# ska-sa/dc_sand

Hardware: AMD Instinct MI355X
Metric: Gcoeff/s (complex weights) 64ant x 1024beam x 32768chan per GPU (higher is better)
Workload: dtype f32

## Files before the change

### dc_sand_amd/csrc/bf_beamform_kernel.inc

```
template <int CH, bool WEIGHTED = false, class... Extra>
__global__ void __launch_bounds__(kBlock) bf_beamform_kernel(const bf_beamform_args a, const Extra... extra)
{
    static_assert(sizeof...(Extra) == (size_t)WEIGHTED && kernel_takes<bf_weights_args, Extra...> == WEIGHTED,
                  "the extra parameter is w, exactly where WEIGHTED is on");
    const bf_weights_args &w = kernel_extra<bf_weights_args>(extra...);
    extern __shared__ __attribute__((aligned(16))) float s_ant[];

    const uint32_t bid = blockIdx.x;
    const uint32_t bg = bid % a.n_bgroups;
    const uint32_t rest = bid / a.n_bgroups;
    const uint32_t cb = rest % a.n_cblocks;
    const uint32_t tex = rest / a.n_cblocks;

    const uint32_t b_local = threadIdx.x & 15u, t_in = threadIdx.x >> 4;
    const uint32_t b = bg * 16u + b_local;
    const uint32_t t = tex * 16u + t_in;
    const bool live = b < a.B;

    const uint32_t fw = a.flags[tex * 16u + (threadIdx.x & 15u)];
    const uint32_t fl = (fw >> 2) == a.epoch ? (fw & 3u) : DCS_CLASS_FAST_LOW;
    const int slow = __syncthreads_or((int)(fl == DCS_CLASS_SLOW));
    const int high = __syncthreads_or((int)(fl != DCS_CLASS_FAST_LOW));

    const float D = a.k.fDenominator, y = a.k.fRcpDenominator;
    const float *tp = a.terms + 2u * ((uint64_t)t * a.A * a.B + (live ? b : 0u));
    const float *gp = WEIGHTED ? w.gn + (live ? b : 0u) : nullptr;
    const uint32_t cbeg = cb * a.chan_per_block;
    const uint32_t cend = min(cbeg + a.chan_per_block, a.C);
    const uint32_t tex_g = a.tex0 + tex;
    const uint32_t words = a.A * 8u;
    const uint32_t sa = min(kAntChunk, a.A);

    for (uint32_t c = cbeg; c < cend; c += CH) {
        float fChan[CH], acc_re[CH], acc_im[CH];
#pragma unroll
        for (int h = 0; h < CH; h++) {
            fChan[h] = (float)(c + h);
            acc_re[h] = 0.0f;
            acc_im[h] = 0.0f;
        }
        for (uint32_t a0 = 0; a0 < a.A; a0 += kAntChunk) {
            const uint32_t na = min(kAntChunk, a.A - a0);
            const uint32_t cw = na * 8u;
            __syncthreads();
#pragma unroll
            for (int h = 0; h < CH; h++) {
                if (c + h < cend) {
                    const uint32_t *src = reinterpret_cast<const uint32_t *>(a.ant) +
                                          ((uint64_t)(c + h) * a.nt16_total + tex_g) * words + (uint64_t)a0 * 8u;
                    for (uint32_t i = threadIdx.x; i < cw; i += kBlock) {
                        const uint32_t w = src[i];
                        const floatx4 f = {(float)(int8_t)(w & 0xffu), (float)(int8_t)((w >> 8) & 0xffu),
                                           (float)(int8_t)((w >> 16) & 0xffu), (float)(int8_t)(w >> 24)};
                        *reinterpret_cast<floatx4 *>(&s_ant[((size_t)h * sa * 8u + i) * 4u]) = f;
                    }
                }
            }
            __syncthreads();

            auto sample = [&](int h, uint32_t al, float &sre, float &sim) {
                const floatx2 v = *reinterpret_cast<const floatx2 *>(&s_ant[(((size_t)h * sa + al) * 16u + t_in) * 2u]);
                sre = v.x;
                sim = v.y;
            };
            if (!slow) {
                dispatch_fast(a.k.uDiv3Exact != 0u, !high, [&](auto div3, auto lowdeg) {
                    auto terms_of = [&](uint32_t al) {
                        if constexpr (WEIGHTED) {
                            const uint64_t i = (uint64_t)(a0 + min(al, na - 1u)) * a.B;
                            const floatx2 k = *reinterpret_cast<const floatx2 *>(tp + 2u * i);
                            return floatx4{k.x, k.y, gp[i], 0.0f};
                        } else {
                            return *reinterpret_cast<const floatx2 *>(tp + 2u * (uint64_t)(a0 + min(al, na - 1u)) * a.B);
                        }
                    };
                    auto products = [&](uint32_t al, const auto kp) {
#pragma unroll
                        for (int h = 0; h < CH; h++) {
                            float re, im, sre, sim;
                            coeff_fast<decltype(div3)::value, decltype(lowdeg)::value>(kp.x, kp.y, fChan[h], D, y, re, im);
                            if constexpr (WEIGHTED) re = kp.z * re, im = kp.z * im;
                            sample(h, al, sre, sim);
                            const float pr = re * sre, pi = im * sim;
                            acc_re[h] = acc_re[h] + pr;
                            acc_im[h] = acc_im[h] + pi;
                        }
                    };
                    decltype(terms_of(0)) qa = terms_of(0), qb = terms_of(1), qc;
                    uint32_t al = 0;
                    for (; al + 2 < na; al += 3) {
                        qc = terms_of(al + 2);
                        products(al, qa);
                        qa = terms_of(al + 3);
                        products(al + 1, qb);
                        qb = terms_of(al + 4);
                        products(al + 2, qc);
                    }
                    if (al < na) products(al, qa);
                    if (al + 1 < na) products(al + 1, qb);
                });
            } else {
#pragma unroll
                for (int h = 0; h < CH; h++) {
                    float are = acc_re[h], aim = acc_im[h];
                    for (uint32_t al = 0; al < na; al++) {
                        const floatx2 kp = *reinterpret_cast<const floatx2 *>(tp + 2u * (uint64_t)(a0 + al) * a.B);
                        float re, im, sre, sim;
                        coeff_slow(kp.x, kp.y, fChan[h], D, re, im);
                        if constexpr (WEIGHTED) {
                            const float g = gp[(uint64_t)(a0 + al) * a.B];
                            re = g * re, im = g * im;
                        }
                        sample(h, al, sre, sim);
                        const float pr = re * sre, pi = im * sim;
                        are = are + pr;
                        aim = aim + pi;
                    }
                    acc_re[h] = are;
                    acc_im[h] = aim;
                }
            }
        }
        if (live) {
#pragma unroll
            for (int h = 0; h < CH; h++) {
                if (c + h < cend) {
                    floatx2 *dst = reinterpret_cast<floatx2 *>(a.beams) +
                                   (((uint64_t)(c + h) * a.nt16_total + tex_g) * a.B + b) * 16u + t_in;
                    if constexpr (WEIGHTED) {
                        const float sb = w.gs[b];
                        *dst = floatx2{sb * acc_re[h], sb * acc_im[h]};
                    } else {
                        *dst = floatx2{acc_re[h], acc_im[h]};
                    }
                }
            }
        }
    }
}
```

### dc_sand_amd/csrc/bf_capi.hip

```cpp

#include <cmath>
#include <cstdio>
#include <cstring>
#include <new>

#include "bf_host.h"

using namespace bf_host;

static_assert(sizeof(dcs_delay_vals) == 16, "delay_vals must be 4 x fp32 (BeamformerParameters.h:61-66)");

namespace {

bool params_ok(const dcs_bf_params *p)
{
    if (!p) return false;
    if (p->nr_channels < 1 || p->nr_channels > (1 << 24)) return false;
    if (p->nr_stations < 1 || p->nr_beams < 1) return false;
    if ((uint64_t)p->nr_stations * (uint64_t)p->nr_beams > 0x7fffffffull) return false;
    if (!(p->sampling_period > 0.0f) || !std::isfinite(p->sampling_period)) return false;
    if (p->fft_size < 1) return false;
    if (p->nr_samples_per_channel < 1 || p->accumulations_before_new_coeffs < 1) return false;
    if (!(p->adc_sample_rate > 0.0) || !std::isfinite(p->adc_sample_rate)) return false;
    const float D = p->sampling_period * (float)p->nr_channels;
// ... 271 lines not shown
        if ((st = (int)bf_warm_module_incoherent()) != 0) break;
        if ((st = (int)bf_warm_module_filterbank()) != 0) break;
        if ((st = (int)bf_warm_module_stokes()) != 0) break;
        if ((st = (int)bf_warm_module_dedisperse()) != 0) break;
        if ((st = (int)bf_warm_module_single_pulse()) != 0) break;
        if ((st = (int)bf_warm_module_correlator()) != 0) break;
        if ((st = (int)bf_warm_module_ddc()) != 0) break;
        const size_t tb = (size_t)c->n_pairs * sizeof(dcs_delay_vals);
        if ((st = (int)hipMalloc((void **)&c->d_table[0], tb)) != 0) break;
        if ((st = (int)hipMalloc((void **)&c->d_table[1], tb)) != 0) break;
        const size_t db = (size_t)kDtSlots * kDtSlotFloats * sizeof(float);
        if ((st = (int)hipMalloc((void **)&c->d_dt, db)) != 0) break;
        if ((st = (int)hipMalloc((void **)&c->d_tt_terms, (size_t)kTermsInline * c->pairs_pad * 8u)) != 0) break;
        if ((st = (int)hipMalloc((void **)&c->d_tt_flags, (size_t)kTermsInline * (c->pairs_pad / 64u) * 4u)) != 0) break;
        if ((st = (int)hipHostMalloc((void **)&c->h_dt, db, hipHostMallocDefault)) != 0) break;
        for (int i = 0; i < kDtSlots && st == 0; i++) st = (int)hipEventCreateWithFlags(&c->dt_ev[i], hipEventDisableTiming);
        if (st != 0) break;
        for (int i = 0; i < kSideStreams && st == 0; i++) {
            st = (int)hipStreamCreateWithFlags(&c->side[i], hipStreamNonBlocking);
            if (st == 0) st = (int)hipEventCreateWithFlags(&c->join_ev[i], hipEventDisableTiming);
        }
        if (st == 0) st = (int)hipEventCreateWithFlags(&c->fork_ev, hipEventDisableTiming);
        if (st != 0) break;
        c->h_dt[0] = 0.0f;
        if ((st = (int)hipMemcpy(c->d_dt, c->h_dt, sizeof(float), hipMemcpyHostToDevice)) != 0) break;
        if ((st = verify_div3(&c->k)) != 0) break;
        c->div3_verified = c->k.uDiv3Exact;
        for (int w = 0; w < 2; w++) {
            bf_kernel_launch l;
            const uint32_t nt_all = (uint32_t)(c->p.nr_samples_per_channel < (int)kDtInline ? c->p.nr_samples_per_channel : (int)kDtInline);
            float dts[kDtInline] = {0.0f};
            if (prepare_tiled(c, w == 1, nullptr, 0.0f, nt_all > 0 ? nt_all : 1u, 0, (uint32_t)c->p.nr_channels, nullptr, &l, dts, false) == DCS_OK && l.func) {
                hipFuncAttributes attr;
                (void)hipFuncGetAttributes(&attr, l.func);
            }
        }
    } while (0);
    if (st != 0) {
        dcs_bf_destroy(c);
        return st;
    }
    *out = c;
    return DCS_OK;
}

int dcs_bf_destroy(dcs_bf_context *c)
{
    if (!c) return DCS_OK;
    (void)hipFree(c->d_table[0]);
    (void)hipFree(c->d_table[1]);
    (void)hipFree(c->d_dt);
    (void)hipFree(c->d_terms);
    (void)hipFree(c->d_flags);
    (void)hipFree(c->d_wnorm);
    (void)hipFree(c->d_wscale);
    (void)hipFree(c->d_tt_terms);
    (void)hipFree(c->d_tt_flags);
    if (c->h_dt) (void)hipHostFree(c->h_dt);
    for (int i = 0; i < kDtSlots; i++)
        if (c->dt_ev[i]) (void)hipEventDestroy(c->dt_ev[i]);
    for (int i = 0; i < kSideStreams; i++) {
        if (c->join_ev[i]) (void)hipEventDestroy(c->join_ev[i]);
        if (c->side[i]) (void)hipStreamDestroy(c->side[i]);
    }
    if (c->fork_ev) (void)hipEventDestroy(c->fork_ev);
    delete c;
    return DCS_OK;
}

int dcs_bf_upload_delays(dcs_bf_context *c, const dcs_delay_vals *table, void *stream)
{
    if (!c || !table) return DCS_ERR_INVALID_ARGUMENT;
    DCS_CHECK_DEVICE(c);
    const int nxt = c->table_set ? (c->cur ^ 1) : c->cur;
    DCS_TRY(hipMemcpyAsync(c->d_table[nxt], table, (size_t)c->n_pairs * sizeof(dcs_delay_vals),
                           hipMemcpyHostToDevice, as_stream(stream)));
    c->cur = nxt;
    c->table_set = true;
    return DCS_OK;
}

int dcs_bf_set_delays_from_global(dcs_bf_context *c, const void *d_global, uint32_t nb_total,
                                  uint32_t beam_offset, void *stream)
{
    if (!c || !d_global) return DCS_ERR_INVALID_ARGUMENT;
    DCS_CHECK_DEVICE(c);
    if ((uint64_t)beam_offset + (uint64_t)c->p.nr_beams > nb_total) return DCS_ERR_OUT_OF_RANGE;
    if ((reinterpret_cast<uintptr_t>(d_global) & 15u) != 0) return DCS_ERR_INVALID_ARGUMENT;
    const int nxt = c->table_set ? (c->cur ^ 1) : c->cur;
    DCS_TRY(bf_launch_gather_beams(c->d_table[nxt], static_cast<const dcs_delay_vals *>(d_global),
                                   (uint32_t)c->p.nr_stations, (uint32_t)c->p.nr_beams, nb_total, beam_offset,
                                   as_stream(stream)));
    c->cur = nxt;
    c->table_set = true;
    return DCS_OK;
}

int dcs_bf_set_tuning(dcs_bf_context *c, const dcs_bf_tuning *t)
{
    if (!c) return DCS_ERR_INVALID_ARGUMENT;
    if (!t) {
        std::memset(&c->tune, 0, sizeof(c->tune));
        c->tune.nontemporal = -1;
        c->tune.xcd_remap = -1;
        c->tune.rows_same_tile = -1;
        c->k.uDiv3Exact = c->div3_verified;
        c->k.fLowDegLimit = 500.0f;
        c->k.uHalfMath = 0u;
        std::memset(c->tuned, 0, sizeof(c->tuned));
        return DCS_OK;
    }
    if (t->form < 0 || t->form > 3) return DCS_ERR_INVALID_ARGUMENT;
    if (t->nontemporal < -1 || t->nontemporal > 1) return DCS_ERR_INVALID_ARGUMENT;
    if (t->chan_per_block < 0 || t->chan_per_block > (1 << 24)) return DCS_ERR_INVALID_ARGUMENT;
    if (t->tiles_per_block != 0 && t->tiles_per_block != 1 && t->tiles_per_block != 2 && t->tiles_per_block != 4)
        return DCS_ERR_INVALID_ARGUMENT;
    if (t->waves_per_block != 0 && t->waves_per_block != 4 && t->waves_per_block != 8 && t->waves_per_block != 16)
        return DCS_ERR_INVALID_ARGUMENT;
    if (t->rows_per_wave < 0 || t->rows_per_wave > 4) return DCS_ERR_INVALID_ARGUMENT;
    if (t->rows_same_tile < -1 || t->rows_same_tile > 1) return DCS_ERR_INVALID_ARGUMENT;
    if (t->xcd_remap < -1 || t->xcd_remap > 1) return DCS_ERR_INVALID_ARGUMENT;
    if (t->math_mode < 0 || t->math_mode > 15) return DCS_ERR_INVALID_ARGUMENT;
    if ((t->math_mode & 4) && t->nontemporal == 0) return DCS_ERR_UNSUPPORTED;
    if (t->wg_per_cu < -1 || t->wg_per_cu == 1 || t->wg_per_cu > 7) return DCS_ERR_INVALID_ARGUMENT;
    c->tune = *t;
    c->k.uDiv3Exact = (t->math_mode & 1) ? 0u : c->div3_verified;
    c->k.fLowDegLimit = (t->math_mode & 2) ? 0.0f : 500.0f;
    c->k.uHalfMath = (t->math_mode & 4) ? 1u : 0u;
    return DCS_OK;
}

int dcs_bf_gpu_utilisation(const dcs_bf_params *p, float kernel_ms, float out[2])
{
    if (!params_ok(p) || !out) return DCS_ERR_INVALID_ARGUMENT;
    const float fRateOfFFTs_Hz = ((float)p->adc_sample_rate) / ((float)p->fft_size);
    const float fTransferTimePerPacket_s = 1 / fRateOfFFTs_Hz;
    float single = (kernel_ms / 1000.0) / (p->nr_samples_per_channel * fTransferTimePerPacket_s);
    float multiple = single / ((float)p->accumulations_before_new_coeffs);
    single *= 4;
    multiple *= 4;
    out[0] = single;
    out[1] = multiple;
    return DCS_OK;
}

#ifdef DCS_PROBES
int dcs_probe_set_knobs(dcs_bf_context *c, const dcs_probe_knobs *k)
{
    if (!c) return DCS_ERR_INVALID_ARGUMENT;
    if (!k) {
        std::memset(&c->probe, 0, sizeof(c->probe));
        return DCS_OK;
    }
    if (k->pace < 0 || k->pace > 4096 || k->fail_at_step < 0) return DCS_ERR_INVALID_ARGUMENT;
    c->probe = *k;
    return DCS_OK;
}
#endif

}
```

### dc_sand_amd/csrc/bf_capi_beamform.hip

```cpp

#include <cstdlib>
#include <cstring>

#include "bf_host.h"

using namespace bf_host;

namespace {

int next_flag_epoch(dcs_bf_context *c, hipStream_t s, uint32_t *epoch)
{
    if (c->flag_epoch >= (1u << 30) - 2u) {
        DCS_TRY(bf_launch_clear_words(c->d_flags, c->terms_steps * (c->pairs_pad / 64u), s));
        c->flag_epoch = 0;
    }
    *epoch = ++c->flag_epoch;
    return DCS_OK;
}

int clear_class_words(dcs_bf_context *c, uint32_t nt, hipStream_t s)
{
    if (!c->flags_cleared) {
        hipStreamCaptureStatus cs = hipStreamCaptureStatusNone;
        DCS_TRY(hipStreamIsCapturing(s, &cs));
        if (cs == hipStreamCaptureStatusNone) return DCS_OK;
        c->flags_cleared = true;
    }
    DCS_TRY(bf_launch_clear_words(c->d_flags, nt, s));
    return DCS_OK;
}

}

namespace bf_host {

int ensure_terms(dcs_bf_context *c, hipStream_t stream)
{
    if (c->d_terms && c->d_flags) return DCS_OK;
    {
        const int cap = refuse_if_capturing(stream);
        if (cap != DCS_OK) return cap;
    }
    if (!c->d_terms) DCS_TRY(hipMalloc((void **)&c->d_terms, (size_t)c->terms_steps * c->pairs_pad * 8u));
    if (!c->d_flags) {
        const size_t nb = (size_t)c->terms_steps * (c->pairs_pad / 64u) * 4u;
        DCS_TRY(hipMalloc((void **)&c->d_flags, nb));
        DCS_TRY(bf_launch_clear_words(c->d_flags, (uint32_t)(nb / 4u), stream));
        c->flag_epoch = 0;
    }
    return DCS_OK;
}

}

namespace {
int ensure_weights(dcs_bf_context *c, hipStream_t stream)
{
    if (c->d_wnorm && c->d_wscale) return DCS_OK;
    {
        const int cap = refuse_if_capturing(stream);
        if (cap != DCS_OK) return cap;
    }
    if (!c->d_wnorm) DCS_TRY(hipMalloc((void **)&c->d_wnorm, (size_t)c->n_pairs * sizeof(float)));
    if (!c->d_wscale) DCS_TRY(hipMalloc((void **)&c->d_wscale, (size_t)c->p.nr_beams * sizeof(float)));
    return DCS_OK;
}

int launch_bform_terms(dcs_bf_context *c, const float *d_weights, uint32_t nt, const float *dt_dev, float dt0, const float *dt_inline,
                       hipStream_t s, uint32_t *epoch)
{
    const int st_ep = next_flag_epoch(c, s, epoch);
    if (st_ep != DCS_OK) return st_ep;
    const int st_clr = clear_class_words(c, nt, s);
    if (st_clr != DCS_OK) return st_clr;
    bf_bform_terms_args ta;
    std::memset(&ta, 0, sizeof(ta));
    ta.delays = c->d_table[c->cur];
    ta.terms = c->d_terms;
    ta.flags = c->d_flags;
    ta.epoch = *epoch;
    ta.dt_dev = dt_dev;
    ta.dt0 = dt0;
    ta.n_pairs = c->n_pairs;
    ta.A = (uint32_t)c->p.nr_stations;
    ta.B = (uint32_t)c->p.nr_beams;
    ta.nt = nt;
    ta.k = c->k;
    const bf_weights_args wa = {d_weights, c->d_wnorm, c->d_wscale};
    return (int)(d_weights ? bf_launch_bform_terms_weighted(ta, wa, dt_inline, s) : bf_launch_bform_terms(ta, dt_inline, s));
}

int beamform_impl(dcs_bf_context *c, const dt_source &src, uint32_t nt, const int8_t *d_antenna,
                  size_t antenna_bytes, float *d_beams, size_t beams_bytes, void *stream, const float *d_weights = nullptr)
{
    if (!c || (nt && (!d_antenna || !d_beams))) return DCS_ERR_INVALID_ARGUMENT;
    DCS_CHECK_DEVICE(c);
    if (nt % 16u) return DCS_ERR_INVALID_ARGUMENT;
    if (!c->table_set) return DCS_ERR_NOT_READY;
    const uint32_t A = (uint32_t)c->p.nr_stations, B = (uint32_t)c->p.nr_beams, C = (uint32_t)c->p.nr_channels;
    if (antenna_bytes < (size_t)A * C * nt * 2u) return DCS_ERR_INVALID_ARGUMENT;
    if (beams_bytes < (size_t)B * C * nt * 2u * sizeof(float)) return DCS_ERR_INVALID_ARGUMENT;
    if ((reinterpret_cast<uintptr_t>(d_antenna) & 3u) || (reinterpret_cast<uintptr_t>(d_beams) & 7u))
        return DCS_ERR_INVALID_ARGUMENT;
    {
        const int st_range = check_dt_range(c, src, nt);
        if (st_range != DCS_OK) return st_range;
    }
    hipStream_t s = as_stream(stream);
    {
        int st_alloc = ensure_terms(c, s);
        if (st_alloc == DCS_OK && d_weights) st_alloc = ensure_weights(c, s);
        if (st_alloc != DCS_OK) return st_alloc;
    }
    const bf_weights_args wa = {d_weights, c->d_wnorm, c->d_wscale};
    uint32_t chunk = c->terms_steps & ~15u;
    if (chunk > kDtSlotFloats) chunk = kDtSlotFloats;
    if (chunk == 0) return DCS_ERR_UNSUPPORTED;
    if (nt > kDtInline) {
        const int cap = refuse_if_capturing(s);
        if (cap != DCS_OK) return cap;
    }
    for (uint32_t done = 0; done < nt;) {
        const uint32_t n = (nt - done) < chunk ? (nt - done) : chunk;
        const float *dt_dev = nullptr;
        float dt_val[kDtInline];
        const bool inl = n <= kDtInline;
        int st = inl ? fill_dt(c, src, done, n, dt_val) : stage_dt(c, src, done, n, s, &dt_dev);
        if (st != DCS_OK) return st;
        uint32_t epoch = 0;
        st = launch_bform_terms(c, d_weights, n, dt_dev, 0.0f, inl ? dt_val : nullptr, s, &epoch);
        if (st != DCS_OK) return st;
        bf_beamform_args a;
        std::memset(&a, 0, sizeof(a));
        a.terms = c->d_terms;
        a.flags = c->d_flags;
        a.epoch = epoch;
        a.ant = d_antenna;
        a.beams = d_beams;
        a.A = A;
        a.B = B;
        a.C = C;
        a.nt16 = n / 16u;
        a.tex0 = done / 16u;
        a.nt16_total = nt / 16u;
        uint32_t cpb = 4;
        while (cpb > 1 && (uint64_t)((B + 15u) / 16u) * ((C + cpb - 1) / cpb) * a.nt16 < 2048u) cpb >>= 1;
        a.chan_per_block = cpb;
        a.k = c->k;
        DCS_TRY(bf_launch_beamform(a, d_weights ? &wa : nullptr, s));
        done += n;
    }
    return DCS_OK;
}
}

namespace {
struct bacc_output {
    enum { kFloat, kInt8, kBlockPower } kind;
    const float *d_weights;
    bf_quant_args quant;
    const bf_complex_args *complex = nullptr;
    size_t block_bytes() const
    {
        return kind == kBlockPower ? sizeof(float) : 32u * (kind == kInt8 ? sizeof(int8_t) : sizeof(float));
    }
    uintptr_t align_mask() const { return kind == kBlockPower ? 3u : 7u; }
};

int beamform_acc_impl(dcs_bf_context *c, const dt_source &src, uint32_t nt, const int8_t *d_antenna, size_t antenna_bytes,
                      void *d_beams, size_t beams_bytes, void *stream, const bacc_output &out = {bacc_output::kFloat, nullptr, {}})
{
    if (!c || (nt && (!d_antenna || !d_beams))) return DCS_ERR_INVALID_ARGUMENT;
    DCS_CHECK_DEVICE(c);
    if (nt % 16u) return DCS_ERR_INVALID_ARGUMENT;
    if (!c->table_set) return DCS_ERR_NOT_READY;
    const uint32_t A = (uint32_t)c->p.nr_stations, B = (uint32_t)c->p.nr_beams, C = (uint32_t)c->p.nr_channels;
    if (A > 256u) return DCS_ERR_UNSUPPORTED;
    if (antenna_bytes < (size_t)A * C * nt * 2u) return DCS_ERR_INVALID_ARGUMENT;
    if (beams_bytes < (size_t)B * C * (nt / 16u) * out.block_bytes()) return DCS_ERR_INVALID_ARGUMENT;
    if ((reinterpret_cast<uintptr_t>(d_antenna) & 15u) || (reinterpret_cast<uintptr_t>(d_beams) & out.align_mask()))
        return DCS_ERR_INVALID_ARGUMENT;
    if ((out.d_weights || out.kind != bacc_output::kFloat || out.complex) && (c->tune.math_mode & 8)) return DCS_ERR_UNSUPPORTED;
    if (nt == 0) return DCS_OK;
    {
        const int st_range = check_dt_range(c, src, 1);
        if (st_range != DCS_OK) return st_range;
    }
    hipStream_t s = as_stream(stream);
    {
        int st_alloc = ensure_terms(c, s);
        if (st_alloc == DCS_OK && out.d_weights) st_alloc = ensure_weights(c, s);
        if (st_alloc != DCS_OK) return st_alloc;
    }
    float dt_coeff = 0.0f;
    int st = fill_dt(c, src, 0, 1, &dt_coeff);
    if (st != DCS_OK) return st;
    uint32_t epoch = 0;
    st = launch_bform_terms(c, out.d_weights, 1, nullptr, dt_coeff, nullptr, s, &epoch);
    if (st != DCS_OK) return st;
    bf_bacc_args a;
    std::memset(&a, 0, sizeof(a));
    a.terms = c->d_terms;
    a.flags = c->d_flags;
    a.epoch = epoch;
    a.ant = d_antenna;
    a.beams = static_cast<float *>(d_beams);
    a.A = A;
    a.B = B;
    a.C = C;
    a.nT16 = nt / 16u;
    a.k = c->k;
    a.fp32_chain = (c->tune.math_mode & 8) ? 1u : 0u;
#ifdef DCS_PROBES
    auto knob = [](int32_t v, const char *env) { const char *e = std::getenv(env); return (uint32_t)(v ? v : (e ? std::atoi(e) : 0)); };
    a.max_rounds = knob(c->probe.bacc_rounds, "DCS_BACC_ROUNDS");
    a.probe = knob(c->probe.bacc_probe, "DCS_BACC_PROBE");
    a.unstaged = knob(c->probe.bacc_unstaged, "DCS_BACC_UNSTAGED");
    a.plain_stores = knob(c->probe.bacc_plain, "DCS_BACC_PLAIN");
    a.no_share = knob(c->probe.bacc_no_share, "DCS_BACC_NOSHARE");
    a.wg_per_cu = knob(c->probe.bacc_wg_per_cu, "DCS_BACC_WPC");
    a.order = knob(c->probe.bacc_order, "DCS_BACC_ORDER");
    a.nbt_force = knob(c->probe.bacc_nbt, "DCS_BACC_NBT");
    a.nw_force = knob(c->probe.bacc_waves, "DCS_BACC_WAVES");
#endif
    const bf_weights_args wa = {out.d_weights, c->d_wnorm, c->d_wscale};
    return (int)bf_launch_beamform_acc(a, out.d_weights ? &wa : nullptr, out.kind == bacc_output::kInt8 ? &out.quant : nullptr,
                                       out.kind == bacc_output::kBlockPower, out.complex, s);
}

}

namespace bf_host {

int generate_and_beamform_weighted_impl(dcs_bf_context *c, const float *dt, uint64_t t0, uint32_t nt, const int8_t *d_antenna,
                                        size_t antenna_bytes, const float *d_weights, float *d_beams, size_t beams_bytes,
                                        void *stream)
{
    if (int e = generate_and_beamform_weighted_args(c, dt, t0, nt, d_weights)) return e;
    return beamform_impl(c, dt_or_index(dt, t0), nt, d_antenna, antenna_bytes, d_beams, beams_bytes, stream, d_weights);
}

int beamform_accumulated_weighted_impl(dcs_bf_context *c, const float *dt_coeff, uint64_t t_coeff, uint32_t nt,
                                       const int8_t *d_antenna, size_t antenna_bytes, const float *d_weights, float *d_beams,
                                       size_t beams_bytes, void *stream)
{
    if (int e = beamform_accumulated_weighted_args(c, nt, d_weights)) return e;
    return beamform_acc_impl(c, dt_or_index(dt_coeff, t_coeff), nt, d_antenna, antenna_bytes, d_beams, beams_bytes,
                             stream, {bacc_output::kFloat, d_weights, {}});
}

int beamform_accumulated_q8_impl(dcs_bf_context *c, const float *dt_coeff, uint64_t t_coeff, uint32_t nt, const int8_t *d_antenna,
                                 size_t antenna_bytes, const float *d_weights, const float *d_quant_gains, int8_t *d_beams_q8,
                                 size_t beams_bytes, unsigned long long *d_clip_count, void *stream)
{
    if (int e = beamform_accumulated_q8_args(c, nt, d_weights, d_quant_gains, d_clip_count)) return e;
    return beamform_acc_impl(c, dt_or_index(dt_coeff, t_coeff), nt, d_antenna, antenna_bytes, d_beams_q8, beams_bytes,
                             stream, {bacc_output::kInt8, d_weights, {d_quant_gains, d_clip_count}});
}

int beamform_accumulated_power_impl(dcs_bf_context *c, const float *dt_coeff, uint64_t t_coeff, uint32_t nt, const int8_t *d_antenna,
                                    size_t antenna_bytes, const float *d_weights, float *d_block_power, size_t power_bytes,
                                    void *stream)
{
    if (int e = beamform_accumulated_power_args(c, nt, d_weights, d_block_power)) return e;
    return beamform_acc_impl(c, dt_or_index(dt_coeff, t_coeff), nt, d_antenna, antenna_bytes, d_block_power, power_bytes,
                             stream, {bacc_output::kBlockPower, d_weights, {}});
}

int beamform_accumulated_complex_impl(dcs_bf_context *c, const float *dt_coeff, uint64_t t_coeff, uint32_t nt, const int8_t *d_antenna,
                                      size_t antenna_bytes, const float *d_weights, uint32_t flags, float *d_beams, size_t beams_bytes,
                                      void *stream)
{
    if (int e = beamform_accumulated_complex_args(c, nt, d_weights, flags, d_beams)) return e;
    const bf_complex_args cx = {flags & DCS_BF_COMPLEX_CONJ};
    return beamform_acc_impl(c, dt_or_index(dt_coeff, t_coeff), nt, d_antenna, antenna_bytes, d_beams, beams_bytes, stream,
                             {bacc_output::kFloat, d_weights, {}, &cx});
}

int beamform_accumulated_complex_power_impl(dcs_bf_context *c, const float *dt_coeff, uint64_t t_coeff, uint32_t nt,
                                            const int8_t *d_antenna, size_t antenna_bytes, const float *d_weights, uint32_t flags,
                                            float *d_block_power, size_t power_bytes, void *stream)
{
    if (int e = beamform_accumulated_complex_power_args(c, nt, d_weights, flags, d_block_power)) return e;
    const bf_complex_args cx = {flags & DCS_BF_COMPLEX_CONJ};
    return beamform_acc_impl(c, dt_or_index(dt_coeff, t_coeff), nt, d_antenna, antenna_bytes, d_block_power, power_bytes, stream,
                             {bacc_output::kBlockPower, d_weights, {}, &cx});
}

int beamform_accumulated_complex_q8_impl(dcs_bf_context *c, const float *dt_coeff, uint64_t t_coeff, uint32_t nt,
                                         const int8_t *d_antenna, size_t antenna_bytes, const float *d_weights, uint32_t flags,
                                         const float *d_quant_gains, int8_t *d_beams_q8, size_t beams_bytes,
                                         unsigned long long *d_clip_count, void *stream)
{
    if (int e = beamform_accumulated_complex_q8_args(c, nt, d_weights, flags, d_quant_gains, d_beams_q8, d_clip_count)) return e;
    const bf_complex_args cx = {flags & DCS_BF_COMPLEX_CONJ};
    return beamform_acc_impl(c, dt_or_index(dt_coeff, t_coeff), nt, d_antenna, antenna_bytes, d_beams_q8, beams_bytes, stream,
                             {bacc_output::kInt8, d_weights, {d_quant_gains, d_clip_count}, &cx});
}
// ... 33 lines not shown
```

### dc_sand_amd/csrc/bf_kernels.h

```cpp
#ifndef DCS_BF_KERNELS_H
#define DCS_BF_KERNELS_H

#include <hip/hip_runtime.h>
#include <stdint.h>

#include "bf_math.h"

struct bf_tiled_args {
    const dcs_delay_vals *delays;
    void *out;
    const float *dt_dev;
    float dt0;
    uint32_t n_pairs;
    uint32_t c0, nc;
    uint32_t nt;
    uint32_t chan_per_block;
    uint32_t n_tile_groups;
    uint32_t n_cblocks;
    uint32_t xcd_remap;
#ifdef DCS_PROBES
    uint32_t pace;
#endif
    dcs_bf_consts k;
    const float *terms;
    const uint32_t *flags;
    uint32_t pairs_pad;
};
constexpr uint32_t kDtInline = 256;
struct bf_tiled_args_inl {
    bf_tiled_args a;
    float dt_inline[kDtInline];
};

struct bf_kernel_launch {
    const void *func;
    dim3 grid, block;
    uint32_t shared;
    bf_tiled_args_inl args;
};
hipError_t bf_prepare_tiled(const bf_tiled_args &a, const float *dt_inline, bool out16, int tiles_per_block,
                            bool nontemporal, bf_kernel_launch *out);

struct bf_terms_args {
    const dcs_delay_vals *delays;
    float *terms;
    uint32_t *flags;
    const float *dt_dev;
    float dt0;
    uint32_t n_pairs, pairs_pad, nt;
    dcs_bf_consts k;
    float dt_inline[8];
    void *out;
    uint32_t c0, nc, out16;
};
constexpr uint32_t kTermsInline = 8;
hipError_t bf_launch_terms(const bf_terms_args &a, hipStream_t stream);
hipError_t bf_prepare_terms(const bf_terms_args &a, const void **func, dim3 *grid, dim3 *block);

struct bf_rows_args {
    const float *terms;
    const uint32_t *flags;
    void *out;
    uint32_t n_pairs, pairs_pad;
    uint32_t c0, nc, nt;
    uint32_t n_colgroups, n_rowgroups;
    uint32_t xcd_remap;
    uint32_t div3;
    uint32_t same_tile;
#ifdef DCS_PROBES
    uint32_t pace;
#endif
    uint32_t lds_pad;
    float D, y;
};
hipError_t bf_launch_rows(const bf_rows_args &a, bool out16, int waves_per_block, int rows_per_wave,
                          bool nontemporal, bool xcd_remap, bool nomath, hipStream_t stream);

struct bf_bform_terms_args {
    const dcs_delay_vals *delays;
    float *terms;
    uint32_t *flags;
    uint32_t epoch;
    const float *dt_dev;
    float dt0;
    uint32_t n_pairs, A, B, nt;
    dcs_bf_consts k;
};
struct bf_bform_terms_args_inl {
    bf_bform_terms_args a;
    float dt_inline[kDtInline];
};
hipError_t bf_launch_bform_terms(const bf_bform_terms_args &a, const float *dt_inline, hipStream_t stream);

struct bf_weights_args {
    const float *g;
    float *gn;
    float *gs;
};
hipError_t bf_launch_clear_words(uint32_t *words, uint32_t n, hipStream_t stream);
hipError_t bf_launch_bform_terms_weighted(const bf_bform_terms_args &a, const bf_weights_args &w, const float *dt_inline,
                                          hipStream_t stream);

struct bf_beamform_args {
    const float *terms;
    const uint32_t *flags;
    uint32_t epoch;
    const int8_t *ant;
    float *beams;
    uint32_t A, B, C;
    uint32_t nt16;
    uint32_t tex0;
    uint32_t nt16_total;
    uint32_t chan_per_block;
    uint32_t n_bgroups, n_cblocks;
    dcs_bf_consts k;
};
hipError_t bf_launch_beamform(const bf_beamform_args &a, const bf_weights_args *w, hipStream_t stream);

struct bf_bacc_args {
    const float *terms;
    const uint32_t *flags;
    uint32_t epoch;
    const int8_t *ant;
    float *beams;
    uint32_t A, B, C, nT16;
    uint32_t fp32_chain;
    uint32_t share_off;
#ifdef DCS_PROBES
    uint32_t max_rounds;
    uint32_t no_share;
    uint32_t plain_stores;
    uint32_t wg_per_cu;
    uint32_t unstaged;
    uint32_t order;
    uint32_t nbt_force;
    uint32_t nw_force;
    uint32_t probe;
#endif
    uint32_t tiles_per_wg, n_bgroups, n_tgroups, nbt_log2, xcd_group;
    dcs_bf_consts k;
};
__host__ __device__ inline uint32_t bf_xcd_grouped(uint32_t w, uint32_t total, uint32_t G)
{
    if (G <= 1u) return w;
    const uint32_t full = total - total % (8u * G);
    if (w >= full) return w;
    const uint32_t x = w & 7u, q = w >> 3;
    return ((q / G) * 8u + x) * G + q % G;
}

#ifdef DCS_PROBES
#define BACC_KNOB(a, f) ((a).f)
#else
#define BACC_KNOB(a, f) 0u
#endif
struct bf_quant_args {
    const float *gains;
    unsigned long long *clips;
};
struct bf_complex_args {
    uint32_t conj;
};
hipError_t bf_launch_beamform_acc(const bf_bacc_args &a, const bf_weights_args *w, const bf_quant_args *q, bool power,
                                  const bf_complex_args *cx, hipStream_t stream);
hipError_t bf_warm_module_mfma();

struct bf_incoh_args {
    const int8_t *ant;
    const float *weights;
    uint32_t *block_power;
    uint64_t rows;
    uint64_t n_groups;
    uint32_t A;
};
hipError_t bf_launch_incoherent_power(const bf_incoh_args &a, hipStream_t stream);
hipError_t bf_warm_module_incoherent();

struct bf_stokes_args {
    const int8_t *beams_x;
    const int8_t *beams_y;
    int32_t *block_stokes;
    uint64_t rows;
    uint64_t n_groups;
    uint32_t nr_stokes;
};
hipError_t bf_launch_stokes_block(const bf_stokes_args &a, hipStream_t stream);
hipError_t bf_warm_module_stokes();

enum bf_integrate_type { BF_INTEGRATE_F32, BF_INTEGRATE_U32 , BF_INTEGRATE_I32 };
struct bf_integrate_args {
    const void *blocks;
    float *out;
    uint64_t total;
    uint32_t bs;
    uint32_t C;
    uint32_t nr_blocks;
    uint32_t n;
    uint32_t accumulate;
};
hipError_t bf_launch_integrate(bf_integrate_type type, const bf_integrate_args &a, hipStream_t stream);
hipError_t bf_warm_module_integrate();

struct bf_dmdelay_args {
    const double *dms;
    int32_t *delays;
    uint64_t total;
    uint32_t C;
    double freq_first, freq_step, sample_time;
};
hipError_t bf_launch_dm_delays(const bf_dmdelay_args &a, hipStream_t stream);
struct bf_dedisp_args {
    const uint8_t *in;
    const int32_t *delays;
    const uint8_t *mask;
    uint32_t *out;
    uint64_t in_spectra, first, out_spectra, first_out;
    uint32_t C, B, T, nr_dm, max_delay;
    uint32_t t_tiles, dm_tiles;
};
hipError_t bf_launch_dedisperse(const bf_dedisp_args &a, hipStream_t stream);
hipError_t bf_warm_module_dedisperse();

struct bf_dtsums_args {
    const uint32_t *plane;
    uint64_t *sums;
    uint64_t plane_spectra, first;
    uint32_t T;
    uint32_t accumulate;
};
hipError_t bf_launch_dm_time_sums(const bf_dtsums_args &a, uint64_t series, hipStream_t stream);
struct bf_boxcar_args {
    const uint32_t *plane;
    const uint32_t *widths;
    uint32_t *peaks;
    uint64_t plane_spectra, first, peak_blocks, first_block;
    uint32_t T, nr_widths, max_width, block_len;
    uint32_t run;
    uint32_t segments;
};
hipError_t bf_launch_boxcar_peaks(const bf_boxcar_args &a, uint64_t series, hipStream_t stream);
struct bf_peaksnr_args {
    const uint32_t *peaks;
    const uint32_t *widths;
    const uint64_t *sums;
    float *snr;
    uint32_t *best;
    uint64_t peak_blocks, first_block, count;
    uint64_t total;
    uint32_t nr_blocks, nr_widths, max_width;
};
hipError_t bf_launch_peak_snr(const bf_peaksnr_args &a, hipStream_t stream);
hipError_t bf_warm_module_single_pulse();

struct bf_corr_args {
    const int8_t *ant;
    int32_t *vis;
    uint64_t NB;
    uint64_t items;
    uint32_t A;
    uint32_t C;
    uint32_t nT16;
    uint32_t n;
    uint32_t nr_vis;
    uint32_t tiles;
    uint32_t st;
    uint32_t units;
// ... 88 lines not shown
```

### dc_sand_amd/csrc/bf_kernels.hip

```cpp

#include "bf_kernels.h"

#include <hip/hip_runtime.h>

#include <cstring>
#include <type_traits>

#include "bf_device.h"

namespace {

template <bool OUT16, int TPB, bool NT, bool ALIGNED, bool NOMATH, int TAG = 0, bool INL = false, bool TERMS = false, bool HALF = false>
__global__ void __launch_bounds__(kBlock) bf_tiled_kernel(const std::conditional_t<INL, bf_tiled_args_inl, bf_tiled_args> args)
{
    const bf_tiled_args &a = [&]() -> const bf_tiled_args & {
        if constexpr (INL)
            return args.a;
        else
            return args;
    }();
    constexpr int PPL = OUT16 ? 4 : 2;
    constexpr int TILE = 64 * PPL;
    constexpr int ROWS = 4 / TPB;
    constexpr uint32_t EB = OUT16 ? 4u : 8u;
// ... 649 lines not shown
}

template <bool OUT16>
hipError_t launch_rows_o(const bf_rows_args &a, int nw, int rpw, bool nt, bool aligned, bool nomath, dim3 grid,
                         hipStream_t stream)
{
    switch (nw) {
    case 4: return launch_rows_w<OUT16, 4>(a, rpw, nt, aligned, nomath, grid, stream);
    case 8: return launch_rows_w<OUT16, 8>(a, rpw, nt, aligned, nomath, grid, stream);
    case 16: return launch_rows_w<OUT16, 16>(a, rpw, nt, aligned, nomath, grid, stream);
    default: return hipErrorInvalidValue;
    }
}

}

hipError_t bf_prepare_terms(const bf_terms_args &a, const void **func, dim3 *grid, dim3 *block)
{
    *func = nullptr;
    if (a.nt == 0 || a.pairs_pad == 0) return hipSuccess;
    if (a.pairs_pad % kBlock || a.nt > 65535u) return hipErrorInvalidValue;
    if (a.dt_dev == nullptr && a.nt > kTermsInline) return hipErrorInvalidValue;
    *func = reinterpret_cast<const void *>(&bf_terms_kernel);
    *grid = dim3(a.pairs_pad / kBlock, a.nt);
    *block = dim3(kBlock);
    return hipSuccess;
}

hipError_t bf_launch_terms(const bf_terms_args &a, hipStream_t stream)
{
    const void *func;
    dim3 grid, block;
    const hipError_t e = bf_prepare_terms(a, &func, &grid, &block);
    if (e != hipSuccess || func == nullptr) return e;
    void *params[] = {const_cast<bf_terms_args *>(&a)};
    return hipLaunchKernel(func, grid, block, params, 0, stream);
}

hipError_t bf_launch_rows(const bf_rows_args &a_in, bool out16, int waves_per_block, int rows_per_wave,
                          bool nontemporal, bool xcd_remap, bool nomath, hipStream_t stream)
{
    bf_rows_args a = a_in;
    if (a.n_pairs == 0 || a.nc == 0 || a.nt == 0) return hipSuccess;
    const uint32_t ppl = out16 ? 4u : 2u;
    const uint32_t cols = 64u * ppl * (a.same_tile ? 1u : (uint32_t)waves_per_block);
    const uint32_t rows = (uint32_t)rows_per_wave * (a.same_tile ? (uint32_t)waves_per_block : 1u);
    a.n_colgroups = (a.n_pairs + cols - 1) / cols;
    a.n_rowgroups = (a.nc + rows - 1) / rows;
    const uint64_t blocks = (uint64_t)a.n_colgroups * a.n_rowgroups * a.nt;
    if (blocks == 0 || blocks > 0x7fffffffull) return hipErrorInvalidValue;
    a.xcd_remap = (xcd_remap && (blocks % 8u) == 0u) ? 1u : 0u;
    const bool aligned = (a.n_pairs % ppl) == 0 && (reinterpret_cast<uintptr_t>(a.out) % 16u) == 0;
    const dim3 grid((uint32_t)blocks);
    return out16 ? launch_rows_o<true>(a, waves_per_block, rows_per_wave, nontemporal, aligned, nomath, grid, stream)
                 : launch_rows_o<false>(a, waves_per_block, rows_per_wave, nontemporal, aligned, nomath, grid, stream);
}

__global__ void __launch_bounds__(kBlock) bf_verify_div3_kernel(float D, float y, uint32_t *mismatches)
{
    const uint32_t i = blockIdx.x * kBlock + threadIdx.x;
    const float x = dcs_bits_f32(0x3f800000u + i);
    const float q = dcs_div_const3(x, D, y);
    const float e = x / D;
    if (dcs_f32_bits(q) != dcs_f32_bits(e)) atomicAdd(mismatches, 1u);
}

hipError_t bf_launch_verify_div3(float D, float y, uint32_t *d_mismatches, hipStream_t stream)
{
    hipLaunchKernelGGL(bf_verify_div3_kernel, dim3((1u << 23) / kBlock), dim3(kBlock), 0, stream, D, y, d_mismatches);
    return hipGetLastError();
}

hipError_t bf_warm_module()
{
    hipFuncAttributes attr;
    return hipFuncGetAttributes(&attr, reinterpret_cast<const void *>(&bf_gather_beams_kernel));
}

__global__ void __launch_bounds__(kBlock) bf_clear_words_kernel(uint32_t *words, const uint32_t n)
{
    const uint32_t i = blockIdx.x * kBlock + threadIdx.x;
    if (i < n) words[i] = 0u;
}

hipError_t bf_launch_clear_words(uint32_t *words, uint32_t n, hipStream_t stream)
{
    if (n == 0) return hipSuccess;
    if (words == nullptr) return hipErrorInvalidValue;
    hipLaunchKernelGGL(bf_clear_words_kernel, dim3((n + kBlock - 1) / kBlock), dim3(kBlock), 0, stream, words, n);
    return hipGetLastError();
}

hipError_t bf_launch_bform_terms(const bf_bform_terms_args &a, const float *dt_inline, hipStream_t stream)
{
    if (a.nt == 0 || a.n_pairs == 0) return hipSuccess;
    if (a.nt > 65535u) return hipErrorInvalidValue;
    const dim3 grid((a.n_pairs + kBlock - 1) / kBlock, a.nt);
    if (dt_inline != nullptr && a.nt > 1u) {
        if (a.nt > kDtInline) return hipErrorInvalidValue;
        bf_bform_terms_args_inl ai;
        ai.a = a;
        std::memcpy(ai.dt_inline, dt_inline, (size_t)a.nt * sizeof(float));
        hipLaunchKernelGGL(bf_bform_terms_kernel<true>, grid, dim3(kBlock), 0, stream, ai);
        return hipGetLastError();
    }
    bf_bform_terms_args b = a;
    if (dt_inline != nullptr) {
        b.dt_dev = nullptr;
        b.dt0 = dt_inline[0];
    } else if (a.dt_dev == nullptr && a.nt != 1u) {
        return hipErrorInvalidValue;
    }
    hipLaunchKernelGGL(bf_bform_terms_kernel<false>, grid, dim3(kBlock), 0, stream, b);
    return hipGetLastError();
}

hipError_t bf_launch_bform_terms_weighted(const bf_bform_terms_args &a, const bf_weights_args &w, const float *dt_inline,
                                          hipStream_t stream)
{
    if (a.nt == 0 || a.n_pairs == 0) return hipSuccess;
    if (a.nt > 65534u) return hipErrorInvalidValue;
    const dim3 grid((a.n_pairs + kBlock - 1) / kBlock, a.nt + 1u);
    if (dt_inline != nullptr && a.nt > 1u) {
        if (a.nt > kDtInline) return hipErrorInvalidValue;
        bf_bform_terms_wargs<true> ai;
        ai.t.a = a;
        std::memcpy(ai.t.dt_inline, dt_inline, (size_t)a.nt * sizeof(float));
        ai.w = w;
        hipLaunchKernelGGL(bf_bform_terms_w_kernel<true>, grid, dim3(kBlock), 0, stream, ai);
        return hipGetLastError();
    }
    bf_bform_terms_wargs<false> b;
    b.t = a;
    b.w = w;
    if (dt_inline != nullptr) {
        b.t.dt_dev = nullptr;
        b.t.dt0 = dt_inline[0];
    } else if (a.dt_dev == nullptr && a.nt != 1u) {
        return hipErrorInvalidValue;
    }
    hipLaunchKernelGGL(bf_bform_terms_w_kernel<false>, grid, dim3(kBlock), 0, stream, b);
    return hipGetLastError();
}

hipError_t bf_launch_beamform(const bf_beamform_args &a_in, const bf_weights_args *w, hipStream_t stream)
{
    bf_beamform_args a = a_in;
    if (a.A == 0 || a.B == 0 || a.C == 0 || a.nt16 == 0) return hipSuccess;
    if (a.chan_per_block == 0) return hipErrorInvalidValue;
    a.n_bgroups = (a.B + 15u) / 16u;
    a.n_cblocks = (a.C + a.chan_per_block - 1) / a.chan_per_block;
    const uint64_t blocks = (uint64_t)a.n_bgroups * a.n_cblocks * a.nt16;
    const uint32_t na = a.A < kAntChunk ? a.A : kAntChunk;
    const int ch = (a.chan_per_block >= 4 && na <= 64u) ? 4 : (a.chan_per_block >= 2 ? 2 : 1);
    const size_t lds = (size_t)na * 32u * sizeof(float) * (size_t)ch;
    if (blocks > 0x7fffffffull) return hipErrorInvalidValue;
    auto launch = [&](auto channels) {
        constexpr int CH = decltype(channels)::value;
        if (w)
            hipLaunchKernelGGL((bf_beamform_kernel<CH, true, bf_weights_args>), dim3((uint32_t)blocks), dim3(kBlock), lds, stream, a, *w);
        else
            hipLaunchKernelGGL((bf_beamform_kernel<CH>), dim3((uint32_t)blocks), dim3(kBlock), lds, stream, a);
    };
    if (ch == 4)
        launch(std::integral_constant<int, 4>{});
    else if (ch == 2)
        launch(std::integral_constant<int, 2>{});
    else
        launch(std::integral_constant<int, 1>{});
    return hipGetLastError();
}
```

### include/dcs_probes.h

```cpp
#ifndef DCS_PROBES_H
#define DCS_PROBES_H

#include "dcs_beamformer.h"

#ifdef __cplusplus
extern "C" {
#endif
#pragma GCC visibility push(default)

struct dcs_probe_knobs {
    int32_t nomath;
    int32_t pace;
    int32_t fail_at_step;
    int32_t bacc_probe;
    int32_t bacc_rounds;
    int32_t bacc_no_share;
    int32_t bacc_plain;
    int32_t bacc_wg_per_cu;
    int32_t bacc_unstaged;
    int32_t bacc_order;
    int32_t bacc_nbt;
    int32_t bacc_waves;
};
int dcs_probe_set_knobs(dcs_bf_context *ctx, const struct dcs_probe_knobs *k);

int dcs_probe_sincos(int which, const float *d_x, size_t n, float *d_sin, float *d_cos, void *stream);
int dcs_probe_fill(void *d_out, size_t bytes, int nontemporal, void *stream);
int dcs_probe_store_pattern(void *d_out, uint32_t rows, uint32_t cols_kib, uint32_t qb, uint32_t rb, int order,
                            int xcd_remap, int nontemporal, uint32_t block_threads, void *stream);

int dcs_probe_one_store(void *d_out, size_t bytes, int store_mode, int stores_per_thread, uint32_t row_bytes, void *stream);

int dcs_probe_reduce(const void *d_in, size_t bytes, uint64_t *checksum, float *max_modulus_dev, void *stream);

int dcs_probe_mfma(int which, uint32_t blocks, uint32_t iters, float *d_out, void *stream);

uint32_t dcs_probe_xcd_grouped(uint32_t w, uint32_t total, uint32_t group);

int dcs_probe_copy(const void *d_in, void *d_out, size_t bytes, int store_mode, int per_thread, void *stream);

#pragma GCC visibility pop
#ifdef __cplusplus
}
#endif
#endif
```

### probes/dcs_probes.py

```python
from __future__ import annotations

import ctypes
from ctypes import POINTER, byref, c_float, c_int, c_size_t, c_uint32, c_uint64, c_void_p

import numpy as np

from .build import LIB, build

_VP = c_void_p
SIGNATURES = [
    ("dcs_probe_sincos", c_int, [c_int, _VP, c_size_t, _VP, _VP, _VP]),
    ("dcs_probe_fill", c_int, [_VP, c_size_t, c_int, _VP]),
    ("dcs_probe_copy", c_int, [_VP, _VP, c_size_t, c_int, c_int, _VP]),
    ("dcs_probe_one_store", c_int, [_VP, c_size_t, c_int, c_int, c_uint32, _VP]),
    ("dcs_probe_reduce", c_int, [_VP, c_size_t, POINTER(c_uint64), POINTER(c_float), _VP]),
    ("dcs_probe_mfma", c_int, [c_int, c_uint32, c_uint32, _VP, _VP]),
    ("dcs_probe_store_pattern", c_int, [_VP, c_uint32, c_uint32, c_uint32, c_uint32, c_int, c_int, c_int, c_uint32, _VP]),
    ("dcs_probe_set_knobs", c_int, [_VP, _VP]),
    ("dcs_probe_xcd_grouped", c_uint32, [c_uint32, c_uint32, c_uint32]),
]

KNOB_FIELDS = ("nomath", "pace", "fail_at_step", "bacc_probe", "bacc_rounds", "bacc_no_share", "bacc_plain", "bacc_wg_per_cu",
               "bacc_unstaged", "bacc_order", "bacc_nbt", "bacc_waves")

_LIB = None


def lib() -> ctypes.CDLL:
    global _LIB
    if _LIB is None:
        if not LIB.exists():
            build()
        L = ctypes.CDLL(str(LIB))
        for name, restype, argtypes in SIGNATURES:
            fn = getattr(L, name)
            fn.restype = restype
            fn.argtypes = argtypes
        _LIB = L
    return _LIB


def _check(status: int, where: str) -> None:
    if status != 0:
        raise RuntimeError(f"{where}: status {status}")


def _s(stream) -> c_void_p:
    if stream is None:
        return c_void_p(None)
    return c_void_p(int(getattr(stream, "handle", stream)))


def tensor_properties(d_ptr, nbytes: int, stream=None) -> tuple[int, float]:
    ck = c_uint64(0)
    dev = c_float(0.0)
    _check(lib().dcs_probe_reduce(c_void_p(int(d_ptr)), int(nbytes), byref(ck), byref(dev), _s(stream)), "dcs_probe_reduce")
    return int(ck.value), float(dev.value)


def sincos(which: int, d_x, n: int, d_sin, d_cos, stream=None) -> None:
    _check(lib().dcs_probe_sincos(int(which), c_void_p(int(d_x)), int(n), c_void_p(int(d_sin)), c_void_p(int(d_cos)), _s(stream)),
           "dcs_probe_sincos")


def fill(d_out, nbytes: int, nontemporal: int = 1, stream=None) -> None:
    _check(lib().dcs_probe_fill(c_void_p(int(d_out)), int(nbytes), int(nontemporal), _s(stream)), "dcs_probe_fill")


def copy(d_in, d_out, nbytes: int, store_mode: int = 1, per_thread: int = 1, stream=None) -> None:
    _check(lib().dcs_probe_copy(c_void_p(int(d_in)), c_void_p(int(d_out)), int(nbytes), int(store_mode), int(per_thread), _s(stream)),
           "dcs_probe_copy")


def store_pattern(d_out, rows, cols_kib, qb, rb, order=0, xcd_remap=0, store_mode=1, block_threads=256, stream=None) -> None:
    _check(lib().dcs_probe_store_pattern(c_void_p(int(d_out)), rows, cols_kib, qb, rb, order, xcd_remap, store_mode, block_threads,
                                         _s(stream)), "dcs_probe_store_pattern")


def one_store(d_out, nbytes, store_mode, stores_per_thread, row_bytes, stream=None) -> None:
    _check(lib().dcs_probe_one_store(c_void_p(int(d_out)), int(nbytes), int(store_mode), int(stores_per_thread), int(row_bytes),
                                     _s(stream)), "dcs_probe_one_store")


def mfma(which: int, blocks: int, iters: int, d_out, stream=None) -> None:
    _check(lib().dcs_probe_mfma(int(which), int(blocks), int(iters), c_void_p(int(d_out)), _s(stream)), "dcs_probe_mfma")


def set_knobs(gen, **knobs) -> None:
    from dc_sand_amd import _lib as product

    if product.LIB_PATH.resolve() != LIB.resolve():
        raise RuntimeError("set_knobs needs the probes build behind the wrappers: run with DCS_LIB_PATH=probes/libdcs_probes.so")
    unknown = set(knobs) - set(KNOB_FIELDS)
    if unknown:
        raise TypeError(f"unknown knob(s) {sorted(unknown)}")
    if not knobs:
        _check(lib().dcs_probe_set_knobs(c_void_p(gen._h), c_void_p(None)), "dcs_probe_set_knobs")
        return
    k = (ctypes.c_int32 * len(KNOB_FIELDS))(*[int(knobs.get(f, 0)) for f in KNOB_FIELDS])
    _check(lib().dcs_probe_set_knobs(c_void_p(gen._h), ctypes.cast(k, c_void_p)), "dcs_probe_set_knobs")
```

Measured before the change: 929.9.

## Prefetch next antenna chunk into registers while computing current chunk

The int8 antenna samples for the next chunk or channel group are now loaded into registers before the current chunk's math runs, so global-load latency overlaps with compute instead of sitting behind a barrier. The per-block __syncthreads_or reductions become per-wavefront ballots, and the terms loads are hoisted ahead of the LDS staging so they also issue earlier. Probe-only knobs for the channel walk and the channel count are added behind DCS_PROBES. The cost is extra registers for the prefetch buffer, which may reduce occupancy. Classifying slow or high per wavefront instead of per block also lets wavefronts in the same block take different paths.

```diff
diff --git a/dc_sand_amd/csrc/bf_beamform_kernel.inc b/dc_sand_amd/csrc/bf_beamform_kernel.inc
--- a/dc_sand_amd/csrc/bf_beamform_kernel.inc
+++ b/dc_sand_amd/csrc/bf_beamform_kernel.inc
@@ -17,19 +17,39 @@
     const uint32_t t = tex * 16u + t_in;
     const bool live = b < a.B;
 
-    const uint32_t fw = a.flags[tex * 16u + (threadIdx.x & 15u)];
-    const uint32_t fl = (fw >> 2) == a.epoch ? (fw & 3u) : DCS_CLASS_FAST_LOW;
-    const int slow = __syncthreads_or((int)(fl == DCS_CLASS_SLOW));
-    const int high = __syncthreads_or((int)(fl != DCS_CLASS_FAST_LOW));
-
-    const float D = a.k.fDenominator, y = a.k.fRcpDenominator;
-    const float *tp = a.terms + 2u * ((uint64_t)t * a.A * a.B + (live ? b : 0u));
-    const float *gp = WEIGHTED ? w.gn + (live ? b : 0u) : nullptr;
     const uint32_t cbeg = cb * a.chan_per_block;
     const uint32_t cend = min(cbeg + a.chan_per_block, a.C);
     const uint32_t tex_g = a.tex0 + tex;
     const uint32_t words = a.A * 8u;
     const uint32_t sa = min(kAntChunk, a.A);
+
+    constexpr int K = CH == 4 ? 2 : (int)(kAntChunk * 8u / kBlock);
+    uint32_t pf[CH * K] = {};
+    auto fetch = [&](uint32_t c, uint32_t a0) {
+        const uint32_t cw = min(kAntChunk, a.A - a0) * 8u;
+#pragma unroll
+        for (int h = 0; h < CH; h++) {
+            if (c + h < cend) {
+                const uint32_t *src = reinterpret_cast<const uint32_t *>(a.ant) +
+                                      ((uint64_t)(c + h) * a.nt16_total + tex_g) * words + (uint64_t)a0 * 8u;
+#pragma unroll
+                for (int k = 0; k < K; k++) {
+                    const uint32_t i = threadIdx.x + (uint32_t)k * kBlock;
+                    if (i < cw) pf[h * K + k] = src[i];
+                }
+            }
+        }
+    };
+    fetch(cbeg, 0u);
+
+    const uint32_t fw = a.flags[tex * 16u + (threadIdx.x & 15u)];
+    const uint32_t fl = (fw >> 2) == a.epoch ? (fw & 3u) : DCS_CLASS_FAST_LOW;
+    const bool slow = __ballot(fl == DCS_CLASS_SLOW) != 0ull;
+    const bool high = __ballot(fl != DCS_CLASS_FAST_LOW) != 0ull;
+
+    const float D = a.k.fDenominator, y = a.k.fRcpDenominator;
+    const float *tp = a.terms + 2u * ((uint64_t)t * a.A * a.B + (live ? b : 0u));
+    const float *gp = WEIGHTED ? w.gn + (live ? b : 0u) : nullptr;
 
     for (uint32_t c = cbeg; c < cend; c += CH) {
         float fChan[CH], acc_re[CH], acc_im[CH];
@@ -42,21 +62,36 @@
         for (uint32_t a0 = 0; a0 < a.A; a0 += kAntChunk) {
             const uint32_t na = min(kAntChunk, a.A - a0);
             const uint32_t cw = na * 8u;
-            __syncthreads();
+            auto terms_of = [&](uint32_t al) {
+                if constexpr (WEIGHTED) {
+                    const uint64_t i = (uint64_t)(a0 + min(al, na - 1u)) * a.B;
+                    const floatx2 k = *reinterpret_cast<const floatx2 *>(tp + 2u * i);
+                    return floatx4{k.x, k.y, gp[i], 0.0f};
+                } else {
+                    return *reinterpret_cast<const floatx2 *>(tp + 2u * (uint64_t)(a0 + min(al, na - 1u)) * a.B);
+                }
+            };
+            decltype(terms_of(0)) qa = terms_of(0), qb = terms_of(1), qc = terms_of(2);
 #pragma unroll
             for (int h = 0; h < CH; h++) {
                 if (c + h < cend) {
-                    const uint32_t *src = reinterpret_cast<const uint32_t *>(a.ant) +
-                                          ((uint64_t)(c + h) * a.nt16_total + tex_g) * words + (uint64_t)a0 * 8u;
-                    for (uint32_t i = threadIdx.x; i < cw; i += kBlock) {
-                        const uint32_t w = src[i];
-                        const floatx4 f = {(float)(int8_t)(w & 0xffu), (float)(int8_t)((w >> 8) & 0xffu),
-                                           (float)(int8_t)((w >> 16) & 0xffu), (float)(int8_t)(w >> 24)};
-                        *reinterpret_cast<floatx4 *>(&s_ant[((size_t)h * sa * 8u + i) * 4u]) = f;
+#pragma unroll
+                    for (int k = 0; k < K; k++) {
+                        const uint32_t i = threadIdx.x + (uint32_t)k * kBlock;
+                        if (i < cw) {
+                            const uint32_t w = pf[h * K + k];
+                            const floatx4 f = {(float)(int8_t)(w & 0xffu), (float)(int8_t)((w >> 8) & 0xffu),
+                                               (float)(int8_t)((w >> 16) & 0xffu), (float)(int8_t)(w >> 24)};
+                            *reinterpret_cast<floatx4 *>(&s_ant[((size_t)h * sa * 8u + i) * 4u]) = f;
+                        }
                     }
                 }
             }
             __syncthreads();
+            const bool more_chunks = a0 + kAntChunk < a.A;
+            const uint32_t c_next = more_chunks ? c : c + CH;
+            const bool has_next = c_next < cend;
+            if (has_next) fetch(c_next, more_chunks ? a0 + kAntChunk : 0u);
 
             auto sample = [&](int h, uint32_t al, float &sre, float &sim) {
                 const floatx2 v = *reinterpret_cast<const floatx2 *>(&s_ant[(((size_t)h * sa + al) * 16u + t_in) * 2u]);
@@ -65,15 +100,6 @@
             };
             if (!slow) {
                 dispatch_fast(a.k.uDiv3Exact != 0u, !high, [&](auto div3, auto lowdeg) {
-                    auto terms_of = [&](uint32_t al) {
-                        if constexpr (WEIGHTED) {
-                            const uint64_t i = (uint64_t)(a0 + min(al, na - 1u)) * a.B;
-                            const floatx2 k = *reinterpret_cast<const floatx2 *>(tp + 2u * i);
-                            return floatx4{k.x, k.y, gp[i], 0.0f};
-                        } else {
-                            return *reinterpret_cast<const floatx2 *>(tp + 2u * (uint64_t)(a0 + min(al, na - 1u)) * a.B);
-                        }
-                    };
                     auto products = [&](uint32_t al, const auto kp) {
 #pragma unroll
                         for (int h = 0; h < CH; h++) {
@@ -86,15 +112,14 @@
                             acc_im[h] = acc_im[h] + pi;
                         }
                     };
-                    decltype(terms_of(0)) qa = terms_of(0), qb = terms_of(1), qc;
                     uint32_t al = 0;
                     for (; al + 2 < na; al += 3) {
-                        qc = terms_of(al + 2);
                         products(al, qa);
                         qa = terms_of(al + 3);
                         products(al + 1, qb);
                         qb = terms_of(al + 4);
                         products(al + 2, qc);
+                        qc = terms_of(al + 5);
                     }
                     if (al < na) products(al, qa);
                     if (al + 1 < na) products(al + 1, qb);
@@ -120,6 +145,7 @@
                     acc_im[h] = aim;
                 }
             }
+            if (has_next) __syncthreads();
         }
         if (live) {
 #pragma unroll
diff --git a/dc_sand_amd/csrc/bf_capi.hip b/dc_sand_amd/csrc/bf_capi.hip
--- a/dc_sand_amd/csrc/bf_capi.hip
+++ b/dc_sand_amd/csrc/bf_capi.hip
@@ -447,7 +447,7 @@
         std::memset(&c->probe, 0, sizeof(c->probe));
         return DCS_OK;
     }
-    if (k->pace < 0 || k->pace > 4096 || k->fail_at_step < 0) return DCS_ERR_INVALID_ARGUMENT;
+    if (k->pace < 0 || k->pace > 4096 || k->fail_at_step < 0 || k->fused_walk < 0 || k->fused_ch < 0) return DCS_ERR_INVALID_ARGUMENT;
     c->probe = *k;
     return DCS_OK;
 }
diff --git a/dc_sand_amd/csrc/bf_capi_beamform.hip b/dc_sand_amd/csrc/bf_capi_beamform.hip
--- a/dc_sand_amd/csrc/bf_capi_beamform.hip
+++ b/dc_sand_amd/csrc/bf_capi_beamform.hip
@@ -144,6 +144,10 @@
         a.tex0 = done / 16u;
         a.nt16_total = nt / 16u;
         uint32_t cpb = 4;
+#ifdef DCS_PROBES
+        if (c->probe.fused_walk > 0) cpb = (uint32_t)c->probe.fused_walk;
+        a.ch_force = (uint32_t)c->probe.fused_ch;
+#endif
         while (cpb > 1 && (uint64_t)((B + 15u) / 16u) * ((C + cpb - 1) / cpb) * a.nt16 < 2048u) cpb >>= 1;
         a.chan_per_block = cpb;
         a.k = c->k;
diff --git a/dc_sand_amd/csrc/bf_kernels.h b/dc_sand_amd/csrc/bf_kernels.h
--- a/dc_sand_amd/csrc/bf_kernels.h
+++ b/dc_sand_amd/csrc/bf_kernels.h
@@ -112,6 +112,9 @@
     uint32_t tex0;
     uint32_t nt16_total;
     uint32_t chan_per_block;
+#ifdef DCS_PROBES
+    uint32_t ch_force;
+#endif
     uint32_t n_bgroups, n_cblocks;
     dcs_bf_consts k;
 };
diff --git a/dc_sand_amd/csrc/bf_kernels.hip b/dc_sand_amd/csrc/bf_kernels.hip
--- a/dc_sand_amd/csrc/bf_kernels.hip
+++ b/dc_sand_amd/csrc/bf_kernels.hip
@@ -825,7 +825,10 @@
     a.n_cblocks = (a.C + a.chan_per_block - 1) / a.chan_per_block;
     const uint64_t blocks = (uint64_t)a.n_bgroups * a.n_cblocks * a.nt16;
     const uint32_t na = a.A < kAntChunk ? a.A : kAntChunk;
-    const int ch = (a.chan_per_block >= 4 && na <= 64u) ? 4 : (a.chan_per_block >= 2 ? 2 : 1);
+    int ch = (a.chan_per_block >= 4 && na <= 64u) ? 4 : (a.chan_per_block >= 2 ? 2 : 1);
+#ifdef DCS_PROBES
+    if (a.ch_force == 1u || a.ch_force == 2u || (a.ch_force == 4u && na <= 64u)) ch = (int)a.ch_force;
+#endif
     const size_t lds = (size_t)na * 32u * sizeof(float) * (size_t)ch;
     if (blocks > 0x7fffffffull) return hipErrorInvalidValue;
     auto launch = [&](auto channels) {
diff --git a/include/dcs_probes.h b/include/dcs_probes.h
--- a/include/dcs_probes.h
+++ b/include/dcs_probes.h
@@ -21,6 +21,8 @@
     int32_t bacc_order;
     int32_t bacc_nbt;
     int32_t bacc_waves;
+    int32_t fused_walk;
+    int32_t fused_ch;
 };
 int dcs_probe_set_knobs(dcs_bf_context *ctx, const struct dcs_probe_knobs *k);
 
diff --git a/probes/dcs_probes.py b/probes/dcs_probes.py
--- a/probes/dcs_probes.py
+++ b/probes/dcs_probes.py
@@ -21,7 +21,7 @@
 ]
 
 KNOB_FIELDS = ("nomath", "pace", "fail_at_step", "bacc_probe", "bacc_rounds", "bacc_no_share", "bacc_plain", "bacc_wg_per_cu",
-               "bacc_unstaged", "bacc_order", "bacc_nbt", "bacc_waves")
+               "bacc_unstaged", "bacc_order", "bacc_nbt", "bacc_waves", "fused_walk", "fused_ch")
 
 _LIB = None
 
```

After: 929.9 (median of 2 runs). Within noise of the previous version (-0.0%).
